# rashanarshad/deconv_api

Measured on AMD Instinct MI355X. Metric: images/sec, VGG16 deconv 224px (block5_conv3 deconvnet, top-4 mosaic), higher is better.
Workload: dtype bf16; 1 GPU; model=vgg16_deconvnet_block5_conv3, global_batch=256, seq_len=224, image_size=224, filters_per_image=4, parallelism=dp1

## Files before the change

deconv_api_amd/csrc/bindings.cpp:

```cpp
#include <torch/extension.h>
#include <ATen/hip/impl/HIPGuardImplMasqueradingAsCUDA.h>
#include <ATen/hip/impl/HIPStreamMasqueradingAsCUDA.h>

#include "jpeg_dec.h"
#include "jpeg_enc.h"
#include "kernels.h"

#include <cstdio>
#include <cstdlib>
#include <cstring>
#include <map>
#include <mutex>
#include <optional>

namespace {

using at::Tensor;

hipStream_t cur_stream() { return c10::hip::getCurrentHIPStreamMasqueradingAsCUDA().stream(); }

void check_cuda(const Tensor& t, const char* name) {
  TORCH_CHECK(t.is_cuda(), name, " must be a GPU tensor");
}

// ... 1329 lines not shown
  TORCH_CHECK(w.scalar_type() == at::kBFloat16 && w.is_contiguous() && w.dim() == 2 && w.size(0) == 64 &&
                  w.size(1) >= 576 && w.size(1) % 64 == 0,
              "conv_unpool_z: w bf16 [64, Kpad >= 576]");
  TORCH_CHECK(w2.scalar_type() == at::kBFloat16 && w2.is_contiguous() && w2.numel() == 32 * 64, "conv_unpool_z: w2 bf16 [32, 64]");
  check_cuda(code, "code");
  check_cuda(w, "w");
  check_cuda(w2, "w2");
  check_cuda(z, "z");
  dv::ConvArgs a{};
  a.N = (int)z.size(0); a.H = a.OH = (int)z.size(1); a.W = a.OW = (int)z.size(2); a.C = 64;
  a.OC = a.OCpad = 64; a.KH = a.KW = 3; a.stride = 1; a.pad_h = a.pad_w = 1;
  a.K = 576; a.Kpad = (int)w.size(1); a.M = a.N * a.H * a.W;
  a.relu = 1; a.relu_in = 1; a.code_div = (int)code_div; a.x_ld = 64; a.out_ld = 32;
  a.dtype = dv::DT_BF16;
  a.x = reinterpret_cast<const uint16_t*>(x.data_ptr());
  a.w = reinterpret_cast<const uint16_t*>(w.data_ptr());
  a.w2 = reinterpret_cast<const uint16_t*>(w2.data_ptr());
  a.code = code.data_ptr<uint8_t>();
  a.out = z.data_ptr();
  a.x_elems = avail_bytes(x) / 2;
  a.out_elems = avail_bytes(z) / 2;
  const int rc = dv::conv3x3_unpool_z_launch(a, cur_stream());
  if (rc == -4) return false;
  check_rc(rc, "conv_unpool_z");
  return true;
}

bool conv_stem_pool(Tensor x, Tensor w1, c10::optional<Tensor> b1, Tensor w2, c10::optional<Tensor> b2, Tensor out,
                    Tensor out_code) {
  check_cuda(x, "x");
  c10::hip::HIPGuardMasqueradingAsCUDA guard(x.device());
  TORCH_CHECK(x.dim() == 4 && x.scalar_type() == at::kBFloat16 && x.is_contiguous() && x.size(3) == 8,
              "conv_stem_pool: x bf16 [N, H, W, 8]");
  const int64_t N = x.size(0), H = x.size(1), W = x.size(2);
  TORCH_CHECK(H % 2 == 0 && W % 2 == 0, "conv_stem_pool: even H, W");
  TORCH_CHECK(out.dim() == 4 && out.scalar_type() == at::kBFloat16 && out.is_contiguous() && out.size(0) == N &&
                  out.size(1) == H / 2 && out.size(2) == W / 2 && out.size(3) == 64,
              "conv_stem_pool: out bf16 [N, H/2, W/2, 64]");
  TORCH_CHECK(out_code.scalar_type() == at::kByte && out_code.is_contiguous() && out_code.numel() == out.numel(),
              "conv_stem_pool: out_code u8 [N, H/2, W/2, 64]");
  TORCH_CHECK(w1.scalar_type() == at::kBFloat16 && w1.is_contiguous() && w1.dim() == 2 && w1.size(0) == 64 &&
                  w1.size(1) >= 96,
              "conv_stem_pool: w1 bf16 [64, Kpad >= 96]");
  TORCH_CHECK(w2.scalar_type() == at::kBFloat16 && w2.is_contiguous() && w2.dim() == 2 && w2.size(0) == 64 &&
                  w2.size(1) >= 576,
              "conv_stem_pool: w2 bf16 [64, Kpad >= 576]");
  for (const auto* b : {&b1, &b2})
    if (b->has_value())
      TORCH_CHECK((*b)->scalar_type() == at::kFloat && (*b)->is_contiguous() && (*b)->numel() >= 64 && (*b)->is_cuda(),
                  "conv_stem_pool: bias fp32 [>= 64] on the device");
  check_cuda(w1, "w1");
  check_cuda(w2, "w2");
  check_cuda(out, "out");
  check_cuda(out_code, "out_code");
  dv::ConvArgs a{};
  a.N = (int)N; a.H = a.OH = (int)H; a.W = a.OW = (int)W; a.C = 64;
  a.OC = a.OCpad = 64; a.KH = a.KW = 3; a.stride = 1; a.pad_h = a.pad_w = 1;
  a.K = 576; a.Kpad = (int)w2.size(1); a.M = (int)(N * H * W);
  a.relu = 1; a.code_div = 1; a.x_ld = 8; a.out_ld = 64;
  a.dtype = dv::DT_BF16;
  a.x = reinterpret_cast<const uint16_t*>(x.data_ptr());
  a.w = reinterpret_cast<const uint16_t*>(w2.data_ptr());
  a.bias = b2.has_value() ? b2->data_ptr<float>() : nullptr;
  a.w2 = reinterpret_cast<const uint16_t*>(w1.data_ptr());
  a.bias2 = b1.has_value() ? b1->data_ptr<float>() : nullptr;
  a.kpad2 = (int)w1.size(1);
  a.out = out.data_ptr();
  a.out_code = out_code.data_ptr<uint8_t>();
  a.x_elems = avail_bytes(x) / 2;
  a.out_elems = avail_bytes(out) / 2;
  dv::g_route = dv::ConvRoute{};
  const int rc = dv::conv3x3_stem_pool_launch(a, cur_stream());
  if (rc == -4) return false;
  check_rc(rc, "conv_stem_pool");
  return true;
}

void zsum3x3(Tensor z, Tensor out, c10::optional<Tensor> stats, int64_t stats_div) {
  check_cuda(z, "z");
  check_cuda(out, "out");
  c10::hip::HIPGuardMasqueradingAsCUDA guard(z.device());
  TORCH_CHECK(z.dim() == 4 && z.scalar_type() == at::kBFloat16 && z.is_contiguous() && z.size(3) == 32,
              "zsum3x3: z bf16 [N, H, W, 32]");
  TORCH_CHECK(out.scalar_type() == at::kFloat && out.is_contiguous() && out.numel() == z.numel() / 32 * 3,
              "zsum3x3: out fp32 [N, H, W, 3]");
  const int N = (int)z.size(0);
  double* st = nullptr;
  if (stats.has_value()) {
    check_cuda(*stats, "stats");
    TORCH_CHECK(stats->scalar_type() == at::kDouble && stats->is_contiguous() && stats_div >= 1 && N % stats_div == 0 &&
                    stats->numel() == 2 * (N / stats_div),
                "zsum3x3: stats fp64 [N/stats_div, 2]");
    check_rc((int)hipMemsetAsync(stats->data_ptr(), 0, stats->numel() * 8, cur_stream()), "stats memset");
    st = stats->data_ptr<double>();
  }
  check_rc(dv::zsum3x3_launch(reinterpret_cast<const uint16_t*>(z.data_ptr()), out.data_ptr<float>(), N,
                              (int)z.size(1), (int)z.size(2), st, (int)stats_div, cur_stream()),
           "zsum3x3");
}

void maxpool2x2(Tensor x, Tensor out, Tensor code) {
  check_cuda(x, "x");
  c10::hip::HIPGuardMasqueradingAsCUDA guard(x.device());
  TORCH_CHECK(x.dim() == 4 && is16(x) && x.is_contiguous(), "maxpool: x NHWC bf16 / fp16");
  const int64_t N = x.size(0), H = x.size(1), W = x.size(2), C = x.size(3);
  TORCH_CHECK(out.scalar_type() == x.scalar_type() && out.is_contiguous() && out.numel() == N * (H / 2) * (W / 2) * C,
              "maxpool: out");
  TORCH_CHECK(code.scalar_type() == at::kByte && code.is_contiguous() && code.numel() == out.numel(), "maxpool: code");
  check_rc(dv::maxpool2x2_launch(reinterpret_cast<const uint16_t*>(x.data_ptr()),
                                 reinterpret_cast<uint16_t*>(out.data_ptr()), code.data_ptr<uint8_t>(), (int)N, (int)H,
                                 (int)W, (int)C, f16(x), cur_stream()),
           "maxpool2x2");
}

void unpool2x2(Tensor p, Tensor code, Tensor out, int64_t code_div, bool relu) {
  check_cuda(p, "p");
  c10::hip::HIPGuardMasqueradingAsCUDA guard(p.device());
  TORCH_CHECK(out.dim() == 4 && is16(out) && out.is_contiguous(), "unpool: out NHWC bf16 / fp16");
  const int64_t N = out.size(0), H = out.size(1), W = out.size(2), C = out.size(3);
  TORCH_CHECK(p.scalar_type() == out.scalar_type() && p.is_contiguous() && p.numel() == N * (H / 2) * (W / 2) * C,
              "unpool: p");
  TORCH_CHECK(code_div >= 1 && N % code_div == 0, "unpool: code_div");
  TORCH_CHECK(code.scalar_type() == at::kByte && code.is_contiguous() && code.numel() == p.numel() / code_div,
              "unpool: code");
  check_rc(dv::unpool2x2_launch(reinterpret_cast<const uint16_t*>(p.data_ptr()), code.data_ptr<uint8_t>(),
                                reinterpret_cast<uint16_t*>(out.data_ptr()), (int)N, (int)H, (int)W, (int)C,
                                (int)code_div, relu ? 1 : 0, cur_stream()),
           "unpool2x2");
}


}

#ifndef DV_SOURCE_HASH
#define DV_SOURCE_HASH "unknown"
#endif
static const char kSourceHash[] = "DV_SOURCE_HASH:" DV_SOURCE_HASH;

PYBIND11_MODULE(TORCH_EXTENSION_NAME, m) {
  m.def("source_hash", [] { return std::string(kSourceHash + 15); }, "sha256 of the sources this binary was built from");
  m.def("subpixel_merge", &subpixel_merge, "strided-conv input gradient from its parity-class parts (+accumulate, emask)");
  m.def("sk_errors", &sk_errors, py::arg("reset") = false,
        "KW3P stream-K hand-offs that timed out since the last reset (their tiles are wrong)");
  m.doc() = "deconv_api_amd gfx950 (MI355X) HIP kernels";
  m.def("conv", &conv, "MFMA implicit-GEMM conv (fwd / unpool-gather / transposed; bf16/pool/f32 epilogues)",
        py::arg("x"), py::arg("w"), py::arg("bias"), py::arg("out"), py::arg("out_code"), py::arg("code"),
        py::arg("mask"), py::arg("geom"), py::arg("amode"), py::arg("epi"), py::arg("impl"),
        py::arg("res") = py::none(), py::arg("emask") = py::none(), py::arg("stats") = py::none(),
        py::arg("stats_div") = 1, py::arg("ucode") = py::none(), py::arg("ucode_div") = 1,
        py::arg("relu_cols") = 0, py::arg("out2") = py::none(), py::arg("split_col") = 0,
        py::arg("obits") = py::none(), py::arg("ebits") = py::none(), py::arg("w_kw3") = py::none());
  m.def("conv_route", &conv_route, "kernel the last conv call on this thread launched (route report)");
  m.def("misc_route", &misc_route, "kernel the last seed_deconv3x3 / maxpool2x2 / unpool2x2 / deprocess_mosaic call chose");
  m.def("conv_bpack", [] { return dv::g_route.bpack != 0; },
        "whether the last conv call on this thread staged its weights from the packed KW3 image (w_kw3)");
  m.def("conv_group_begin", &conv_group_begin, "start recording groupable small-problem convs (this thread)");
  m.def("conv_group_pause", [](bool p) { g_group_paused = p; }, "suspend / resume recording (dependent convs)");
  m.def("conv_group_end", &conv_group_end, "launch the recorded convs as grouped kernels; returns the launch count");
  m.def("dma_tune", [](int64_t cfg, int64_t ks) { dv::conv_dma_tune((int)cfg, (int)ks); },
        "force the LDS-DMA conv tile config / split-K factor (0 = automatic); tuning only");
  m.def("pool", &pool, "k x k max/avg pooling forward/backward", py::arg("in"), py::arg("out"), py::arg("idx"),
        py::arg("kind"), py::arg("dir"), py::arg("geom"), py::arg("bias") = py::none(), py::arg("relu") = false,
        py::arg("accumulate") = false);
  m.def("subpixel_scatter", &subpixel_scatter, "input gradient of a stride-s 1x1 conv from its GEMM result");
  m.def("sumsq_core", &sumsq_core, "DeepDream loss: per-image partial sums of squares over the core");
  m.def("stem_conv", &stem_conv, "strided few-channel stem conv (direct VALU kernels), fwd (dir 0) / dgrad (dir 1)");
  m.def("sumsq_core_bwd", &sumsq_core_bwd, "DeepDream loss gradient (+ optional addend)", py::arg("x"),
        py::arg("scale"), py::arg("gx"), py::arg("b"), py::arg("addend") = py::none(), py::arg("part") = py::none());
  m.def("tile_gather", &tile_gather, "tiled DeepDream: rolled tile gather into the 16-bit network input", py::arg("x"),
        py::arg("xin"), py::arg("plan"), py::arg("shift"), py::arg("rank"), py::arg("world"), py::arg("k0") = 0);
  m.def("tile_pack", &tile_pack, "tiled DeepDream: owned-pixel gradient pack + unit loss / sum|g| tail", py::arg("g"),
        py::arg("pack"), py::arg("plan"), py::arg("lpart"), py::arg("lcoef"), py::arg("ucap"), py::arg("rank"),
        py::arg("world"), py::arg("k0") = 0);
  m.def("tile_update", &tile_update, "tiled DeepDream: normalize + update the image from every rank's packs");
  m.def("tile_pack_elems", &tile_pack_elems);
  m.def("dream_update", &dream_update, "fused DeepDream normalize + update + next network input");
  m.def("octave_resize", &octave_resize, "DeepDream octave transition: corner-aligned bilinear resize of (a + b - c)",
        py::arg("a"), py::arg("b"), py::arg("c"), py::arg("y"), py::arg("yin") = py::none());
  m.def("stem7_fwd", &stem7_fwd, "ResNet-50 conv1 forward (7x7 / 2, RGB -> 64) on the tap-paired MFMA kernel");
  m.def("stem_dgrad_fused", &stem_dgrad_fused, "fused GEMM + col2im input gradient of a 7x7/2 RGB stem conv");
  m.def("col2im", &col2im, "col2im of a strided few-channel conv's input gradient");
  m.def("jpeg_data_urls", &jpeg_data_urls, "native JPEG + base64/quote data URLs (GIL released)");
  m.def("softmax_rows", &softmax_rows, "row softmax (classifier head)");
  m.def("paced_copy", &paced_copy, "bench: CU-occupying copy paced to a link bandwidth (all-gather interference model)");
  m.def("jpeg_gpu", &jpeg_gpu, "GPU baseline JPEG scans of uint8 [B,H,W,3] (restart per MCU row)");
  m.def("data_url_b64decode", &data_url_b64decode, "data URL payload -> bytes (lenient base64, GIL released)");
  m.def("url_unquote_plus", &url_unquote_plus, "unquote_plus of an ASCII str -> bytes (GIL released)");
  m.def("jpeg_gpu_header", &jpeg_gpu_header, "SOI..SOS of the GPU encoder's streams");
  m.def("jpeg_gpu_max_width", &dv::jpeg_gpu_max_width, "widest image the GPU encoder takes");
  m.def("jpeg_gpu_data_urls", &jpeg_gpu_data_urls, "GPU scans -> data URLs (host base64, GIL released)");
  m.def("jpeg_encode", &jpeg_encode, "native baseline JPEG encode (GIL released)");
  m.def("jpeg_parse_coeffs", &jpeg_parse_coeffs, "baseline JPEG bytes -> None | (header, int16 coefficients) (GIL released)");
  m.def("data_url_parse_coeffs", &data_url_parse_coeffs, "data URL -> (payload | None, None | parsed coefficients)");
  m.def("jpeg_dec_batch", &jpeg_dec_batch, "GPU JPEG decode of a batch: coefficients -> RGB, two launches");
  m.def("channel_sum", &channel_sum);
  m.def("topk_pos", &topk_pos);
  m.def("seed_deconv3x3", &seed_deconv3x3);
  m.def("seed_map", &seed_map, "deconvnet seed maps (all / max, optional max-unpool for pool targets)");
  m.def("deprocess_mosaic", &deprocess_mosaic, py::arg("recon"), py::arg("out"), py::arg("tiles"), py::arg("reverse"),
        py::arg("stats") = py::none());
  m.def("resize_preprocess", &resize_preprocess);
  m.def("resize_batch", &resize_batch, "variable-size batch resize (+preprocess) from one staged blob");
  m.def("preprocess_u8", &preprocess_u8, "resized RGB u8 -> caffe-preprocessed bf16 network input");
  m.def("maxpool2x2", &maxpool2x2);
  m.def("unpool2x2", &unpool2x2);
  m.def("conv_stem_pool", &conv_stem_pool, "fused VGG16 stem: conv 8->64 -> conv 64->64 -> 2x2 max-pool + switches");
  m.def("conv_unpool_z", &conv_unpool_z, "unpool -> conv3x3 64->64 -> ReLU -> per-tap products of the next 64->3 conv");
  m.def("zsum3x3", &zsum3x3, "9-tap shift-add of a per-tap product map (+ ReLU, per-image stats)");
  m.attr("ARCH") = "gfx950";
}
```

deconv_api_amd/csrc/conv_halo_stream.hip:

```cpp
#include "common.h"
#include "kernels.h"

#include <cstdlib>
#include <cstring>

namespace dv {

namespace {

constexpr int HS_TH = 16, HS_TW = 32;
constexpr int HS_HH = HS_TH + 2, HS_HW = HS_TW + 2;
constexpr int HS_PS = 80;
constexpr int HS_HSLOTS = HS_HH * HS_HW * 5;
constexpr int HS_HI = (HS_HSLOTS + 511) / 512;
constexpr int HS_HBUF = HS_HI * 8 * 1024;
constexpr uint32_t HS_OOB = 0x80000000u;

typedef int hs_i32x4 __attribute__((ext_vector_type(4)));

__device__ __forceinline__ void hs_dma16(const hs_i32x4& rsrc, const uint8_t* lds_dst, uint32_t voff) {
  asm volatile("s_mov_b32 m0, %0\n\ts_nop 0\n\tbuffer_load_dwordx4 %1, %2, 0 offen lds"
               :
               : "s"(__builtin_amdgcn_readfirstlane((uint32_t)(uintptr_t)lds_dst)), "v"(voff), "s"(rsrc)
               : "memory");
// ... 552 lines not shown
      issue_w(k + 2);
      const uint8_t* wb = ring + (k % RING) * BSLOT + wrd;
      const int kh = t / 3, kw = t % 3;
      v8 wf[FN], pf[4];
#pragma unroll
      for (int j = 0; j < FN; ++j) wf[j] = *reinterpret_cast<const v8*>(wb + j * 16 * 64);
#pragma unroll
      for (int i = 0; i < 4; ++i) {
        const int p = (4 * wave + i + kh) * H16_HW + px + kw;
        pf[i] = *reinterpret_cast<const v8*>(hb + p * 64 + ((q ^ h16_swz(p)) << 4));
      }
      __builtin_amdgcn_s_setprio(1);
#pragma unroll
      for (int i = 0; i < 4; ++i)
#pragma unroll
        for (int j = 0; j < FN; ++j) acc[i][j] = mfma16x16x32<DT>(wf[j], pf[i], acc[i][j]);
      __builtin_amdgcn_s_setprio(0);
      if constexpr (UNPOOL) {
        if (t == STEPS_PER_CHUNK - 1 && c + 1 < nch) {
          hs_wait<STEPS_PER_CHUNK * BI>();
          __builtin_amdgcn_s_barrier();
          expand((c + 1) & 1);
          asm volatile("s_waitcnt lgkmcnt(0)" ::: "memory");
        }
      }
    }
  }
  }
  hs_wait<0>();

  const int ox = tx0 + px;
  float4 bv[FN];
#pragma unroll
  for (int j = 0; j < FN; ++j)
    bv[j] = a.bias ? *reinterpret_cast<const float4*>(a.bias + 16 * j + 4 * q) : make_float4(0.f, 0.f, 0.f, 0.f);
  const float lo = a.relu ? 0.f : -INFINITY;
  uint16_t* out = reinterpret_cast<uint16_t*>(a.out);
  if constexpr (POOL) {
    const int PH = H >> 1, PW = W >> 1;
#pragma unroll
    for (int i = 0; i < 4; i += 2) {
      const long long prow = ((long long)n * PH + ((ty0 >> 1) + 2 * wave + (i >> 1))) * PW + (ox >> 1);
      const bool st = (px & 1) == 0;
#pragma unroll
      for (int j = 0; j < FN; ++j) {
        const int oc = 16 * j + 4 * q;
        const float b4[4] = {bv[j].x, bv[j].y, bv[j].z, bv[j].w};
        float best[4];
        uint32_t codes = 0;
#pragma unroll
        for (int r = 0; r < 4; ++r) {
          float w4[4];
#pragma unroll
          for (int d = 0; d < 2; ++d) {
            const float v = to_f<DT>(from_f<DT>(fmaxf(acc[i + d][j][r] + b4[r], lo)));
            w4[2 * d] = v;
            w4[2 * d + 1] = __int_as_float(__builtin_amdgcn_mov_dpp(__float_as_int(v), 0xB1, 0xF, 0xF, false));
          }
          float m = w4[0];
          uint32_t cc = 0;
#pragma unroll
          for (int e = 1; e < 4; ++e)
            if (w4[e] > m) {
              m = w4[e];
              cc = e;
            }
          best[r] = m;
          codes |= cc << (8 * r);
        }
        if (st && oc < a.OC && DV_BOUNDS(prow * a.out_ld + oc, 4, a.out_elems, "hs16 pool out")) {
          *reinterpret_cast<uint2*>(out + prow * a.out_ld + oc) =
              make_uint2(pack2<DT>(best[0], best[1]), pack2<DT>(best[2], best[3]));
          *reinterpret_cast<uint32_t*>(a.out_code + prow * a.OC + oc) = codes;
        }
      }
    }
    return;
  }
  if constexpr (LEPI) {
    __syncthreads();
    constexpr int ROWB = OCT * 2, CPR = OCT / 8;
    uint8_t* wreg = smem + wave * 64 * ROWB;
    static_assert(4 * 64 * ROWB <= (int)sizeof(smem), "LDS epilogue slices");
#pragma unroll
    for (int i = 0; i < 4; ++i)
#pragma unroll
      for (int j = 0; j < FN; ++j) {
        const float v0 = fmaxf(acc[i][j][0] + bv[j].x, lo), v1 = fmaxf(acc[i][j][1] + bv[j].y, lo);
        const float v2 = fmaxf(acc[i][j][2] + bv[j].z, lo), v3 = fmaxf(acc[i][j][3] + bv[j].w, lo);
        const int ch = 2 * j + (q >> 1);
        *reinterpret_cast<uint2*>(wreg + (i * 16 + px) * ROWB + ((ch ^ (px & (CPR - 1))) << 4) + (q & 1) * 8) =
            make_uint2(pack2<DT>(v0, v1), pack2<DT>(v2, v3));
      }
    asm volatile("s_waitcnt lgkmcnt(0)" ::: "memory");
    constexpr int PPI = 64 / CPR, NT = 64 / PPI;
    const int pc = lane % CPR;
    uint4 em[NT];
#pragma unroll
    for (int t = 0; t < NT; ++t) {
      const int lp = t * PPI + lane / CPR;
      const int lc = pc ^ (lp & (CPR - 1));
      const long long pix = ((long long)n * a.OH + ty0 + 4 * wave + (lp >> 4)) * a.OW + tx0 + (lp & 15);
      em[t] = make_uint4(0x3C003C00u, 0x3C003C00u, 0x3C003C00u, 0x3C003C00u);
      if (a.ebits && lc * 8 < a.OC)
        em[t].x = a.ebits[pix * a.ebits_ld + lc];
      else if (a.emask && lc * 8 < a.OC && DV_BOUNDS(pix * a.emask_ld + lc * 8, 8, a.emask_elems, "hs16 emask"))
        em[t] = *reinterpret_cast<const uint4*>(a.emask + pix * a.emask_ld + lc * 8);
    }
#pragma unroll
    for (int t = 0; t < NT; ++t) {
      const int lp = t * PPI + lane / CPR;
      const int lc = pc ^ (lp & (CPR - 1));
      const long long pix = ((long long)n * a.OH + ty0 + 4 * wave + (lp >> 4)) * a.OW + tx0 + (lp & 15);
      uint4 v = *reinterpret_cast<const uint4*>(wreg + lp * ROWB + pc * 16);
      if (a.ebits) {
        v = mask_bits8(v, em[t].x);
      } else if (a.emask) {
        v.x = mask_pos_pk(v.x, em[t].x);
        v.y = mask_pos_pk(v.y, em[t].y);
        v.z = mask_pos_pk(v.z, em[t].z);
        v.w = mask_pos_pk(v.w, em[t].w);
      }
      if (lc * 8 < a.OC && DV_BOUNDS(pix * a.out_ld + lc * 8, 8, a.out_elems, "hs16 out")) {
        *reinterpret_cast<uint4*>(out + pix * a.out_ld + lc * 8) = v;
        if (a.obits) a.obits[pix * a.obits_ld + lc] = (uint8_t)pos_bits8(v);
      }
    }
    return;
  }
#pragma unroll
  for (int i = 0; i < 4; ++i) {
    const int oy = ty0 + 4 * wave + i;
    const long long pix = ((long long)n * a.OH + oy) * a.OW + ox;
    uint16_t* orow = out + pix * a.out_ld;
    uint2 em[FN];
#pragma unroll
    for (int j = 0; j < FN; ++j) {
      const int oc = 16 * j + 4 * q;
      em[j] = make_uint2(0x3C003C00u, 0x3C003C00u);
      if (a.emask && oc < a.OC && DV_BOUNDS(pix * a.emask_ld + oc, 4, a.emask_elems, "hs16 emask"))
        em[j] = *reinterpret_cast<const uint2*>(a.emask + pix * a.emask_ld + oc);
    }
#pragma unroll
    for (int j = 0; j < FN; ++j) {
      const int oc = 16 * j + 4 * q;
      if (oc >= a.OC) continue;
      const float v0 = fmaxf(acc[i][j][0] + bv[j].x, lo), v1 = fmaxf(acc[i][j][1] + bv[j].y, lo);
      const float v2 = fmaxf(acc[i][j][2] + bv[j].z, lo), v3 = fmaxf(acc[i][j][3] + bv[j].w, lo);
      if (DV_BOUNDS(pix * a.out_ld + oc, 4, a.out_elems, "hs16 out"))
        *reinterpret_cast<uint2*>(orow + oc) =
            make_uint2(mask_pos_pk(pack2<DT>(v0, v1), em[j].x), mask_pos_pk(pack2<DT>(v2, v3), em[j].y));
    }
  }
}

static int hs_ring() {
  static int v = [] {
    const char* e = dv_ab_env("DV_HS_RING");
    const int r = e ? std::atoi(e) : 3;
    return r == 4 || r == 5 ? r : 3;
  }();
  return v;
}

#define HS_LAUNCH(DT_, OCT_, POOL_)                                                                    \
  do {                                                                                                 \
    if (ring == 5)                                                                                     \
      hipLaunchKernelGGL((conv3x3_hs_kernel<DT_, OCT_, POOL_, 5>), grid, block, 0, s, a, tx, ty);      \
    else if (ring == 4)                                                                                \
      hipLaunchKernelGGL((conv3x3_hs_kernel<DT_, OCT_, POOL_, 4>), grid, block, 0, s, a, tx, ty);      \
    else                                                                                               \
      hipLaunchKernelGGL((conv3x3_hs_kernel<DT_, OCT_, POOL_, 3>), grid, block, 0, s, a, tx, ty);      \
  } while (0)

int conv3x3_hs_launch(const ConvArgs& a, int epi, hipStream_t s, bool* lepi_used) {
  if (lepi_used) *lepi_used = false;
  if (dv_ab_env("DV_NO_HS") != nullptr) return -4;
  if ((a.OCpad == 192 || a.OCpad == 256) && a.OC > 128 && epi == CONV_E_BF16 && dv_ab_env("DV_NO_HS_SPLIT") == nullptr) {
    ConvArgs a1 = a, a2 = a;
    a1.OC = 128;
    a1.OCpad = 128;
    a2.OC = a.OC - 128;
    a2.OCpad = a.OCpad - 128;
    a2.w = a.w + (long long)128 * a.Kpad;
    a2.bias = a.bias ? a.bias + 128 : nullptr;
    a2.out = reinterpret_cast<uint16_t*>(a.out) + 128;
    a2.out_elems = a.out_elems - 128;
    if (a.emask) {
      a2.emask = a.emask + 128;
      a2.emask_elems = a.emask_elems - 128;
    }
    a1.obits = a2.obits = nullptr;
    a1.ebits = a2.ebits = nullptr;
    if (a2.OC % 4 != 0) return -4;
    const int r1 = conv3x3_hs_launch(a1, epi, s);
    if (r1 < 0) return r1;
    const int r2 = conv3x3_hs_launch(a2, epi, s);
    g_route.flags |= CR_F_OCSPLIT;
    return r2;
  }
  const bool geom = a.KH == 3 && a.KW == 3 && a.stride == 1 && a.pad_h == a.pad_w && a.pad_h >= 0 && a.pad_h <= 2 &&
                    a.OH == a.H + 2 * a.pad_h - 2 && a.OW == a.W + 2 * a.pad_w - 2 && a.OH > 0 && a.OW > 0;
  if (!geom || a.C % 32 != 0 || a.x_ld % 8 != 0 || (a.OCpad != 64 && a.OCpad != 128) || a.relu_in || a.accumulate ||
      a.mask || a.code || a.res || a.ws || a.stats || a.ucode || a.relu_cols > 0 || a.out_ld % 4 != 0 ||
      (reinterpret_cast<uintptr_t>(a.out) & 7) || (reinterpret_cast<uintptr_t>(a.x) & 15) ||
      (reinterpret_cast<uintptr_t>(a.bias) & 15) ||
      (a.emask && (a.emask_ld % 4 != 0 || (reinterpret_cast<uintptr_t>(a.emask) & 7))) ||
      (long long)a.Kpad < 9LL * a.C || (long long)a.H * a.W * a.x_ld * 2 > 0x7FFFFFF0LL)
    return -4;
  const bool pool = epi == CONV_E_POOL;
  if (!pool && epi != CONV_E_BF16) return -4;
  if (pool && (a.pad_h != 1 || a.emask || a.H % 2 || a.W % 2 || a.out_code == nullptr || a.OC % 4 ||
               a.dtype != DT_BF16 || (reinterpret_cast<uintptr_t>(a.out_code) & 3)))
    return -4;
  if (a.OH % 16 == 0 && a.OW % 16 == 0 && a.OC % 4 == 0 && dv_ab_env("DV_NO_HS16") == nullptr) {
    const int t16x = a.OW / 16, t16y = a.OH / 16;
    const long long n16 = (long long)a.N * t16x * t16y;
    if (n16 <= 0 || n16 > 0x7fffffffLL) return -2;
    const dim3 g16((unsigned)n16), b16(256);
#define HS16(DT_, OCT_, POOL_, LEPI_)                                                                            \
  hipLaunchKernelGGL((conv3x3_hs16_kernel<DT_, OCT_, POOL_, false, OCT_ == 64 ? 3 : 1, LEPI_>), g16, b16, 0, s, a, t16x, \
                     t16y)
    const char* he = dv_ab_env("DV_HS16_EPI");
    const bool lepi = !pool && !(he && std::strcmp(he, "reg") == 0) && a.OC % 8 == 0 && a.out_ld % 8 == 0 &&
                      !(reinterpret_cast<uintptr_t>(a.out) & 15) &&
                      (!a.emask || (a.emask_ld % 8 == 0 && !(reinterpret_cast<uintptr_t>(a.emask) & 15)));
    if (lepi_used) *lepi_used = lepi;
    route_set(CR_HS16, 0, a.OCpad, 0, 0, pool ? CR_E_POOL : (lepi ? CR_E_LDS : CR_E_REG));
    if (pool) {
      if (a.OCpad == 128) HS16(DT_BF16, 128, true, false);
      else HS16(DT_BF16, 64, true, false);
    } else if (a.dtype == DT_F16) {
      if (a.OCpad == 128) {
        if (lepi) HS16(DT_F16, 128, false, true);
        else HS16(DT_F16, 128, false, false);
      } else {
        if (lepi) HS16(DT_F16, 64, false, true);
        else HS16(DT_F16, 64, false, false);
      }
    } else {
      if (a.OCpad == 128) {
        if (lepi) HS16(DT_BF16, 128, false, true);
        else HS16(DT_BF16, 128, false, false);
      } else {
        if (lepi) HS16(DT_BF16, 64, false, true);
        else HS16(DT_BF16, 64, false, false);
      }
    }
#undef HS16
    return (int)hipGetLastError();
  }
  const int tx = (a.OW + HS_TW - 1) / HS_TW, ty = (a.OH + HS_TH - 1) / HS_TH;
  const long long nwg = (long long)a.N * tx * ty;
  if (nwg <= 0 || nwg > 0x7fffffffLL) return -2;
  const dim3 grid((unsigned)nwg), block(512);
  const int ring = hs_ring();
  const char* he = dv_ab_env("DV_HS16_EPI");
  const bool lepi = !pool && ring == 3 && !(he && std::strcmp(he, "reg") == 0) && a.OC % 8 == 0 && a.out_ld % 8 == 0 &&
                    !(reinterpret_cast<uintptr_t>(a.out) & 15) &&
                    (!a.emask || (a.emask_ld % 8 == 0 && !(reinterpret_cast<uintptr_t>(a.emask) & 15)));
  if (lepi_used) *lepi_used = lepi;
  route_set(CR_HS32, 0, a.OCpad, 0, 0, pool ? CR_E_POOL : (lepi ? CR_E_LDS : CR_E_REG));
#define HS_LEPI(DT_, OCT_, NB1_) \
  hipLaunchKernelGGL((conv3x3_hs_kernel<DT_, OCT_, false, 3, NB1_, true>), grid, block, 0, s, a, tx, ty)
  if (pool) {
    if (a.OCpad == 128) HS_LAUNCH(DT_BF16, 128, true);
    else HS_LAUNCH(DT_BF16, 64, true);
  } else if (a.C == 32 && a.OCpad == 64) {
    if (a.dtype == DT_F16) {
      if (lepi) HS_LEPI(DT_F16, 64, true);
      else hipLaunchKernelGGL((conv3x3_hs_kernel<DT_F16, 64, false, 3, true>), grid, block, 0, s, a, tx, ty);
    } else {
      if (lepi) HS_LEPI(DT_BF16, 64, true);
      else hipLaunchKernelGGL((conv3x3_hs_kernel<DT_BF16, 64, false, 3, true>), grid, block, 0, s, a, tx, ty);
    }
  } else if (lepi) {
    if (a.dtype == DT_F16) {
      if (a.OCpad == 128) HS_LEPI(DT_F16, 128, false);
      else HS_LEPI(DT_F16, 64, false);
    } else {
      if (a.OCpad == 128) HS_LEPI(DT_BF16, 128, false);
      else HS_LEPI(DT_BF16, 64, false);
    }
  } else if (a.dtype == DT_F16) {
    if (a.OCpad == 128) HS_LAUNCH(DT_F16, 128, false);
    else HS_LAUNCH(DT_F16, 64, false);
  } else {
    if (a.OCpad == 128) HS_LAUNCH(DT_BF16, 128, false);
    else HS_LAUNCH(DT_BF16, 64, false);
  }
#undef HS_LEPI
  return (int)hipGetLastError();
}

int conv3x3_stem_pool_launch(const ConvArgs& a, hipStream_t s) {
  if (a.KH != 3 || a.KW != 3 || a.stride != 1 || a.pad_h != 1 || a.pad_w != 1 || a.C != 64 || a.OC != 64 ||
      a.OCpad != 64 || a.x_ld != 8 || a.H != a.OH || a.W != a.OW || a.H % 16 || a.W % 16 || a.H <= 0 || a.W <= 0 ||
      a.N <= 0 || a.dtype != DT_BF16 || a.w2 == nullptr || a.kpad2 < 96 || a.Kpad < 9 * 64 || a.out_code == nullptr ||
      a.out_ld != 64 || a.relu != 1 || a.relu_in || a.accumulate || a.mask || a.code || a.res || a.emask || a.ws ||
      a.ucode || (reinterpret_cast<uintptr_t>(a.x) & 15) || (reinterpret_cast<uintptr_t>(a.out) & 7) ||
      (reinterpret_cast<uintptr_t>(a.out_code) & 3) || (reinterpret_cast<uintptr_t>(a.w2) & 15) ||
      (long long)a.H * a.W * 8 * 2 > 0x7FFFFFF0LL)
    return -4;
  const int tx = a.W / 16, ty = a.H / 16;
  const long long nwg = (long long)a.N * tx * ty;
  if (nwg > 0x7fffffffLL) return -2;
  route_set(CR_HS16, 0, 64, 0, 0, CR_E_POOL);
  g_route.cfg = 1;
  hipLaunchKernelGGL((conv3x3_hs16_kernel<DT_BF16, 64, true, false, 3, false, true>), dim3((unsigned)nwg), dim3(256), 0,
                     s, a, tx, ty);
  return (int)hipGetLastError();
}

}
```

deconv_api_amd/csrc/kernels.h:

```cpp
#pragma once
#include <hip/hip_runtime_api.h>
#include <stdint.h>

#include <cstdlib>

static inline bool dv_ablations_on() {
  const char* on = std::getenv("DV_ABLATIONS");
  return on != nullptr && on[0] == '1' && on[1] == 0;
}
static inline const char* dv_ab_env(const char* name) { return dv_ablations_on() ? std::getenv(name) : nullptr; }

namespace dv {

enum ConvAMode : int {
  CONV_A_FWD = 0,
  CONV_A_UNPOOL = 1,
  CONV_A_TRANSPOSE = 2,
};
enum ConvEpi : int {
  CONV_E_BF16 = 0,
  CONV_E_POOL = 1,
  CONV_E_F32 = 2,
};

enum { DT_BF16 = 0, DT_F16 = 1 };

struct ConvArgs {
  const uint16_t* x;
  long long x_ld;
  const uint16_t* mask;
  long long mask_ld;
  const uint8_t* code;
  int code_div;
  const uint16_t* w;
  const float* bias;
  void* out;
  long long out_ld;
  uint8_t* out_code;
  int N, H, W, C;
  int OH, OW, OC, OCpad;
  int KH, KW, stride, pad_h, pad_w;
  int K, Kpad;
  int M;
  int m_base;
  int relu, relu_in, accumulate;
  int dtype;
  const uint16_t* res;
  long long res_ld;
  const uint16_t* emask;
  long long emask_ld;
  int vec_epi;
  int epi_batch;
  float* ws;
  int ksplit;
  double* stats;
  int stats_div;
  const uint8_t* ucode;
  int ucode_div;
  long long x_elems, out_elems, res_elems, emask_elems;
  int relu_cols;
  void* out2;
  long long out2_ld;
  int split_col;
  long long out2_elems;
  const uint16_t* w2;
  int pool_t;
  float* skw;
  unsigned* skflag;
  int skslots;
  unsigned* skerr;
  uint8_t* obits;
  long long obits_ld;
  const uint8_t* ebits;
  long long ebits_ld;
  const float* bias2;
  int kpad2;
  const uint16_t* wp;
  long long wp_elems;
};
constexpr long long kSkSlotFloats = 256LL * 256LL;
constexpr int kSkMaxWg = 1024;

constexpr int kGroupMax = 4;
struct ConvGroup {
  ConvArgs p[kGroupMax];
  int start[kGroupMax + 1];
  int tiles_n[kGroupMax];
  int n;
};

enum ConvRouteKind : int {
  CR_NONE = 0, CR_IGEMM, CR_HALO_V1, CR_HALO_V2, CR_POOL_V3, CR_C8_STREAM, CR_HS16, CR_HS32, CR_PW, CR_DMA,
  CR_KW3, CR_KW3P, CR_GROUP,
};
enum ConvRouteEpi : int {
  CR_E_NONE = 0, CR_E_REG, CR_E_LDS, CR_E_UNPOOL, CR_E_POOL, CR_E_STRIPS, CR_E_PERSIST,
  CR_E_POOL_T, CR_E_POOL_LDS,
};
enum ConvRouteFlag : int {
  CR_F_SK = 1,
  CR_F_OCSPLIT = 2,
  CR_F_TAIL = 4,
  CR_F_UNPOOL = 8,
  CR_F_RELU_COPY = 16,
  CR_F_MASK = 32,
};
struct ConvRoute {
  int kind, bm, bn, stages, ksplit, epi, flags, m_base, cfg;
  int bpack;
};
extern __thread ConvRoute g_route;
static inline void route_set(int kind, int bm, int bn, int stages, int ksplit, int epi, int flags = 0) {
  g_route = ConvRoute{kind, bm, bn, stages, ksplit, epi, (g_route.flags & (CR_F_UNPOOL | CR_F_RELU_COPY)) | flags, 0, 0};
}

extern __thread const char* g_misc_route;

int conv_igemm_launch(const ConvArgs& a, int amode, int epi, hipStream_t stream);
int conv_dma_launch(const ConvArgs& a, int amode, int epi, hipStream_t stream);
int conv_dma_splitk(const ConvArgs& a);
void conv_dma_tune(int cfg, int ks);
int splitk_reduce_launch(const ConvArgs& a, int epi, hipStream_t stream);
int conv_dma_group_cfg(const ConvArgs& a, int amode, int epi);
int conv_dma_group_launch(const ConvArgs* ps, int n, int amode, int epi, hipStream_t stream);
int stem_conv_fwd_launch(const uint16_t* x, const float* w, const float* bias, uint16_t* y, int N, int H, int W,
                         int OH, int OW, int C, int cr, int cout, int k, int stride, int pad, int relu, long long x_ld,
                         long long y_ld, int dtype, hipStream_t s);
int stem_conv_dgrad_launch(const uint16_t* gy, const float* w, uint16_t* gx, int N, int H, int W, int OH, int OW,
                           int C, int cr, int cout, int k, int stride, int pad, long long gy_ld, long long gx_ld,
                           int dtype, hipStream_t s);
int conv_pw_launch(const ConvArgs& a, hipStream_t stream);

int channel_sum_launch(const uint16_t* x, float* sums, int N, int HW, int C, int f16, hipStream_t s);
int topk_pos_launch(const float* v, int* idx, float* val, int N, int C, int k, hipStream_t s);
int seed_deconv3x3_launch(const float* S, const int* f, const uint16_t* wt, uint16_t* out,
                          int B, int H, int W, int Cin, int F, int f16, hipStream_t s);
int deprocess_mosaic_launch(const float* recon, uint8_t* out, int B, int H, int W, int tiles,
                            int reverse_channels, hipStream_t s);
int recon_stats_launch(const float* x, double* stats, long long per_group, int groups, hipStream_t s);
int deprocess_apply_launch(const float* recon, const double* stats, uint8_t* out, int B, int H, int W, int tiles,
                           int reverse_channels, hipStream_t s);
int resize_preprocess_launch(const uint8_t* img, int B, int Hs, int Ws, uint16_t* out, int OH, int OW,
                             int Cpad, int mode, int f16, hipStream_t s);
int resize_batch_launch(const uint8_t* blob, const long long* table, int B, void* out, int OH, int OW, int Cpad,
                        int fmt, hipStream_t s);
int preprocess_u8_launch(const uint8_t* in, uint16_t* out, long long P, int Cpad, int f16, hipStream_t s);
int maxpool2x2_launch(const uint16_t* x, uint16_t* out, uint8_t* code, int N, int H, int W, int C,
                      int f16, hipStream_t s);
int seed_map_launch(const uint16_t* out4, const int* idx, const uint8_t* code, float* S, int BK, int K, int H, int W,
                    int C, int mode, int f16, hipStream_t s);
int unpool2x2_launch(const uint16_t* p, const uint8_t* code, uint16_t* out, int N, int H, int W,
                     int C, int code_div, int relu, hipStream_t s);

}

namespace dv {
int subpixel_merge_launch(const uint16_t* const* p, const int* hc, const int* wc, const int* ld, const uint16_t* emask,
                          uint16_t* gx, int N, int H, int W, int C, int s, int acc, int dtype, hipStream_t st);
int subpixel_scatter_launch(const uint16_t* E, const uint16_t* emask, uint16_t* gx, int N, int H, int W, int C, int OH,
                            int OW, int s, int dtype, hipStream_t st);
int pool_launch(int kind, int dir, const uint16_t* in, uint16_t* out, uint8_t* idx, int N, int H, int W, int C,
                int OH, int OW, int k, int s, int pad, int dtype, hipStream_t st, long long x_ld = 0,
                long long y_ld = 0, const float* bias = nullptr, int relu = 0, int acc = 0);
int dream_update_launch(const uint16_t* g, float* x, uint16_t* xin, float* gpart, int gparts, const float* lpart,
                        const float* lcoef, int L, int lparts, uint8_t* done, float* loss, float step, float max_loss,
                        int N, int H, int W, int dtype, hipStream_t s);
int octave_resize_launch(const float* a, const float* b, const float* c, float* y, uint16_t* yin, int N, int Hs, int Ws, int Hd, int Wd,
                         int dtype, hipStream_t s);
int tile_gather_launch(const float* x, uint16_t* xin, const int* plan, const int* shift, int units, int rank, int world,
                       int k0, int H, int W, int Th, int Tw, int dtype, hipStream_t s);
int tile_pack_launch(const uint16_t* g, uint16_t* pack, const int* plan, const float* lpart, const float* lcoef, int L,
                     int lparts, int units, int ucap, int rank, int world, int k0, int Th, int Tw, int dtype, hipStream_t s);
long long tile_pack_elems(int ucap, int Th, int Tw);
int tile_update_launch(const uint16_t* packs, long long pack_elems, int units_per_rank, const int* plan, int nunits,
                       const int* shift, float* x, uint8_t* done, float* loss, float step, float max_loss, int world,
                       int H, int W, int Th, int Tw, int dtype, hipStream_t s);
int sumsq_core_launch(const uint16_t* x, float* part, int parts, int N, int H, int W, int C, int b, int dtype,
                      hipStream_t s);
int sumsq_core_bwd_launch(const uint16_t* x, const float* scale, const uint16_t* addend, uint16_t* gx, int N, int H, int W, int C, int b,
                          int dtype, hipStream_t s);
int sumsq_core_fused_launch(const uint16_t* x, const float* scale, const uint16_t* addend, uint16_t* gx, float* part,
                            int parts, int N, int H, int W, int C, int b, int dtype, hipStream_t s);
struct Col2ImGeom {
  int N, H, W, OH, OW, KH, KW, stride, pad_h, pad_w, Cr, J_ld;
};
int col2im_launch(const uint16_t* cols, uint16_t* gx, const Col2ImGeom& g, int dtype, hipStream_t s);
struct StemDgradGeom {
  int N, H, W, OH, OW, C, KH, KW, stride, pad, Cr, w_rows, w_ld;
};
int stem7_fwd_launch(const uint16_t* x, const uint16_t* w, const float* bias, uint16_t* y, int N, int H, int W, int OH,
                     int OW, int relu, int dtype, hipStream_t s);
int stem_dgrad_fused_launch(const uint16_t* gy, const uint16_t* mask, const uint16_t* wb, uint16_t* gx,
                            const StemDgradGeom& g, int dtype, hipStream_t s);
long long jpeg_gpu_ws_bytes(int B, int H, int W);
long long jpeg_gpu_out_cap(int H, int W);
int jpeg_gpu_max_width();
int jpeg_gpu_launch(const uint8_t* rgb, int B, int H, int W, const void* tables, void* ws, uint8_t* packed,
                    long long* off, hipStream_t s);
int jpeg_dec_launch(uint8_t* blob, long long blob_bytes, const int* table, int B, int total_blocks, int total_items,
                    hipStream_t s);
int softmax_rows_launch(const float* x, float* y, int M, int N, hipStream_t s);
int paced_copy_launch(const void* src, long long src_bytes, void* dst, long long bytes, int channels, double gbs,
                      hipStream_t s);
int conv3x3_halo_launch(const ConvArgs& a, int unpool, int epi, hipStream_t s, bool* stats_done = nullptr);
int conv3x3_pool_v3_launch(const ConvArgs& a, hipStream_t s);
int conv3x3_unpool_z_launch(const ConvArgs& a, hipStream_t s);
int zsum3x3_launch(const uint16_t* z, float* out, int N, int H, int W, double* stats, int stats_div, hipStream_t s);
int conv3x3_c8_stream_launch(const ConvArgs& a, hipStream_t s);
int conv3x3_stem_pool_launch(const ConvArgs& a, hipStream_t s);
int conv3x3_hs_launch(const ConvArgs& a, int epi, hipStream_t s, bool* lepi_used = nullptr);
}
```

deconv_api_amd/knobs.py:

```python
from __future__ import annotations

import os
from typing import Optional

RUNTIME = {
    "DV_NO_KW3_SK": "stream-K off for KW3P convs (the recovery named by the hand-off timeout error, ops/conv.py)",
    "DV_POOL_SPLIT": "layers whose pool runs as a separate vectorized kernel (config 2 option, docs/KERNELS.md)",
    "DV_STEM_FUSE": "kill switch of the fused VGG16 stem (conv -> conv -> pool in one launch)",
    "DV_FUSED_TAIL": "kill switch of the fused deconvnet tail (unpool -> conv -> per-tap products)",
    "DV_CONV_IMPL": "conv kernel policy for tests / bring-up (auto | dma | igemm | halo)",
    "DV_CONV_GROUP": "grouped launch of independent small convs (DeepDream), 0 = per-conv launches",
    "DV_TILE_COLLECTIVE": "run the multi-rank tiled-DeepDream code path on a 1-rank RCCL group (rehearsal)",
    "DV_TILE_CHUNKS": "tile units per rank split into this many chunks whose all-gathers overlap compute",
    "DV_TILE_CHUNK_STREAMS": "streams the chunks of a tiled step fork onto",
    "DV_TILE_LOCAL_CHUNKS": "chunks per rank when the dream is not collective (one GPU)",
    "DV_TILE_CAPTURE_COLL": "capture the tiled octave's all-gathers inside its hipGraph (0: per-step graphs)",
    "DV_DREAM_GRAPHS": "hipGraph replay of DeepDream steps (0: eager, debugging)",
    "DV_DREAM_OCTAVE_GRAPH": "one hipGraph per octave incl. all steps (0: one graph per step)",
    "DV_FAULT": "fault injection for the failover tests (utils/faults.py)",
    "DV_ROCTX": "roctx ranges around engine stages (utils/tracing.py)",
    "DV_MAX_PIXELS": "decoded-pixel cap of a request image (codec/image.py)",
    "DV_FORCE_PG": "create a real process group at world 1 (exercises RCCL collectives on one GPU)",
    "DV_INGEST_DIR": "directory of the front-end <-> GPU-owner Unix sockets (serve/ingest.py)",
    "DV_ABLATIONS": "honour the ABLATION switches below (tools / variant tests only)",
}

ABLATION = {
    "DV_KW3": "KW3 kernel off / forced, ahead of the small-problem tiles too (tests: small shapes with many borders)",
    "DV_KW3_VAR": "KW3 main-loop variant (profiles/kw3_variants_r3.txt, kw3_staging_ablation_r5.txt)",
    "DV_KW3_TILE": "KW3P tile shape (profiles/kw3_ab_r4.txt)",
    "DV_KW3_SK": "stream-K on every eligible grid, not only short ones (profiles/kw3_skall_ab_r5.txt)",
    "DV_KW3P_EPI": "register-layout 8-B epilogue instead of the LDS-staged 16-B one (profiles/kw3_epi_ab_r5.txt)",
    "DV_KW3_BPACK": "0: KW3 weights from the strided w_gemm, not the packed image (profiles/kw3_bpack_ab_r7.txt)",
    "DV_KW3P_NO_PRE": "no step-1 DMA ahead of the epilogue (profiles/kw3_pre_ab_r5.txt)",
    "DV_KW3P_UNP_NT": "plain instead of non-temporal unpool stores (profiles/bench_c2_r5_unp_nt_ab.txt)",
    "DV_NO_KW3P_UNPOOL": "unpool-out conv-downs off KW3P (profiles/kw3_store_ablation_r5.txt)",
    "DV_ALLOW_WRONG_ABLATION": "timing-only variants whose outputs are wrong (tools/kw3_ab.py, tools/tail_ab.py)",
    "DV_NO_AUTO_CFG": "size-based DMA tile choice only (docs/KERNELS.md)",
    "DV_SMALL_TILE_KMIN": "K threshold of the 64x64 small-problem tile",
    "DV_NO_SPLITK": "split-K off, latched at the first DMA conv (tools/small_conv_latency.py; tests: dma_tune(0, 1))",
    "DV_NO_SMALL_SPLITK": "small-problem split-K off",
    "DV_SMALL_SPLITK_MN": "M x N ceiling of the small-problem split-K",
    "DV_NO_POOL_T": "per-element pool-epilogue stores (profiles/bench_c2_r4_pool_t_ab.txt)",
    "DV_POOL_EPI": "pool epilogue variant (profiles/bench_c2_r5_pool_epi_ab.txt)",
    "DV_NO_VEC_EPI": "scalar conv epilogue",
    "DV_NO_EPI_BATCH": "per-row epilogue batching off (profiles/dream_c3_r2_epi_batch*.log)",
    "DV_NO_C8_STREAM": "first-layer row-streaming kernel off",
    "DV_HS_MIN_W": "smallest map side routed to the halo-stream kernels",
    "DV_HS_EMASK_OFF": "masked dgrads back on the DMA kernel",
    "DV_HS_PAD_OFF": "pad != 1 convs off the halo-stream kernels",
    "DV_NO_HS": "halo-stream kernels off",
    "DV_NO_HS16": "16x16-tile halo-stream kernel off",
    "DV_NO_HS_SPLIT": "192/256-channel convs not split into halo-stream halves",
    "DV_HS_RING": "halo-stream ring depth",
    "DV_HS16_EPI": "register-layout epilogue of hs16 (profiles/bench_c2_r5_hs16_epi_ab.txt)",
    "DV_TAIL_V": "fused-tail schedule bits (profiles/bench_c2_r5_tail_v_ab.txt)",
    "DV_STREAM_P": "row-streaming kernel prefetch depth",
    "DV_NO_POOL_UNROLL": "generic k x k pooling loop (profiles/dream_r4_maxpool_bwd_s2_ab.txt)",
    "DV_NO_PW": "persistent 1x1 kernel off (tools/pw_bench.py)",
    "DV_PW_MIN_TILES": "tiles below which 1x1 convs stay on the DMA kernel (profiles/dream_r4_pw_min_tiles.txt)",
    "DV_PW_WG_PER_CU": "persistent 1x1 workgroups per CU",
    "DV_NO_STREAM_PROBE": "plain pool streams instead of probed / high-priority ones (runtime/streams.py)",
    "DV_DREAM_OCTAVE_RESIZE": "torch octave resize instead of the HIP kernel (profiles/dream_c3_r4_octave_resize_ab.txt)",
    "DV_DREAM_FUSED": "fused step tail off",
    "DV_DREAM_FUSED_LOSS": "fused loss off",
    "DV_DREAM_TAPS": "tap-split stride-2 dgrads (profiles/dream_c5_r2_taps.log)",
    "DV_DREAM_SPLIT": "concurrent sub-batches per DeepDream batch (profiles/dream_c3_split_sweep_r2.txt)",
    "DV_RELU_BITS": "1-bit ReLU masks off (profiles/dream_c5_r5_relu_bits_ab.txt)",
    "DV_SUBPIXEL": "sub-pixel scatter for stride-2 1x1 dgrads (profiles/kstats_c5_r2_subpixel.txt)",
    "DV_STEM_FUSED": "InceptionV3 stem fusion (profiles/dream_c3_r2_stem*.log)",
    "DV_STEM_DIRECT": "direct stride-2 stem gradient (profiles/dream_c5_r3_stem_ab.txt)",
    "DV_STEM7": "ResNet conv1 tap-paired kernel (profiles/dream_c5_r5_stem7_ab.txt)",
    "DV_COL2IM": "LDS-tiled col2im of the RGB stem gradient",
    "DV_STRIDED_DIRECT_GFLOP": "size threshold of the direct strided dgrad",
    "DV_MERGE_B1": "merged Inception branch-head GEMMs (profiles/dream_c3_r2_merge_b1.txt)",
    "DV_INCEPTION_FUSED": "one-node Inception blocks (profiles/dream_c3_merged.log)",
}

BUILD = {
    "DV_HIP_CHECK": "launch-status check macro (csrc/common.h), not an environment variable",
    "DV_DEBUG": "-DDV_DEBUG=1 build: device bounds checks (python -m deconv_api_amd._build --debug)",
    "DV_BOUNDS": "the bounds-check macro of DV_DEBUG builds (csrc/common.h)",
    "DV_SOURCE_HASH": "sha256 of csrc + flags embedded in _C (_build.py provenance)",
    "DV_OFFLOAD_ARCH": "offload arch of the in-tree build (gfx950)",
    "DV_AUTOBUILD": "ops/native.py: build (or rebuild a stale) _C in-tree on first use",
    "DV_SKIP_PROVENANCE": "ops/native.py: load a _C built from other sources (scratch builds in tools)",
    "DV_S": "kernel-local macro (conv_smalln.hip), not an environment variable",
    "DV_S2": "kernel-local macro (conv_smalln.hip), not an environment variable",
    "DV_P": "kernel-local macro (conv_smalln.hip), not an environment variable",
}


def config_names():
    import dataclasses

    from .config import Config

    return {"DV_" + f.name.upper() for f in dataclasses.fields(Config)}


def ablations_on() -> bool:
    return os.environ.get("DV_ABLATIONS", "") == "1"


def ablation(name: str, default: Optional[str] = None) -> Optional[str]:
    assert name in ABLATION, f"{name} is not a registered ablation switch (knobs.py)"
    return os.environ.get(name, default) if ablations_on() else default
```

Measured before the change: 7905 images/s.

## Add persistent fused stem conv kernel that prefetches next tile's RGB and weights

Adds a persistent version of the fused VGG stem (conv1_1 + conv1_2 + 2x2 maxpool with codes). The grid is capped at two workgroups per CU, and each workgroup walks many tiles. The first-layer weights and biases stay in registers across tiles. The next tile's RGB halo and the weight ring are DMA-prefetched while the current tile computes. This is meant to cut per-workgroup setup and the launch tail, at the cost of a fixed grid and larger LDS use. It is on by default unless bias2 is misaligned or the DV_HS16_PERSIST env var is 0.

```diff
diff --git a/deconv_api_amd/csrc/bindings.cpp b/deconv_api_amd/csrc/bindings.cpp
--- a/deconv_api_amd/csrc/bindings.cpp
+++ b/deconv_api_amd/csrc/bindings.cpp
@@ -1505,6 +1505,8 @@
         py::arg("obits") = py::none(), py::arg("ebits") = py::none(), py::arg("w_kw3") = py::none());
   m.def("conv_route", &conv_route, "kernel the last conv call on this thread launched (route report)");
   m.def("misc_route", &misc_route, "kernel the last seed_deconv3x3 / maxpool2x2 / unpool2x2 / deprocess_mosaic call chose");
+  m.def("conv_route_flags", [] { return dv::g_route.flags; },
+        "ConvRouteFlag bits of the last conv / conv_stem_pool call on this thread (64: the persistent fused stem)");
   m.def("conv_bpack", [] { return dv::g_route.bpack != 0; },
         "whether the last conv call on this thread staged its weights from the packed KW3 image (w_kw3)");
   m.def("conv_group_begin", &conv_group_begin, "start recording groupable small-problem convs (this thread)");
diff --git a/deconv_api_amd/csrc/conv_halo_stream.hip b/deconv_api_amd/csrc/conv_halo_stream.hip
--- a/deconv_api_amd/csrc/conv_halo_stream.hip
+++ b/deconv_api_amd/csrc/conv_halo_stream.hip
@@ -728,6 +728,212 @@
             make_uint2(mask_pos_pk(pack2<DT>(v0, v1), em[j].x), mask_pos_pk(pack2<DT>(v2, v3), em[j].y));
     }
   }
+}
+
+namespace {
+constexpr int SP_BSLOT = 64 * 64 * 3;
+constexpr int SP_RGB = 2 * 4 * 1024;
+constexpr int SP_SMEM = 2 * H16_HBUF + 2 * SP_BSLOT + SP_RGB;
+static_assert(SP_SMEM <= 80 * 1024, "persistent stem: 2 workgroups per CU");
+}
+
+__global__ void __launch_bounds__(256, 2) conv3x3_stem_persist_kernel(const ConvArgs a, int tiles_x, int tiles_y, int ntiles) {
+  constexpr int DT = DT_BF16;
+  constexpr int C = 64, FN = 4;
+  typedef typename Vec8<DT>::type v8;
+  __shared__ __attribute__((aligned(16))) uint8_t smem[SP_SMEM];
+  uint8_t* halo = smem;
+  uint8_t* ring = smem + 2 * H16_HBUF;
+  uint8_t* rgb = ring + 2 * SP_BSLOT;
+
+  const int tid = threadIdx.x, lane = tid & 63;
+  const int wave = __builtin_amdgcn_readfirstlane(tid >> 6);
+  const int q = lane >> 4, px = lane & 15;
+  const int H = a.H, W = a.W;
+  const int per_img = tiles_x * tiles_y;
+  const int G = (int)gridDim.x;
+  int tile = xcd_remap(blockIdx.x, G);
+  if (tile >= ntiles) return;
+
+  const long long img = (long long)H * W * 8;
+  const hs_i32x4 wr = hs_rsrc(a.w, (long long)a.OCpad * a.Kpad * 2);
+  uint32_t woff[3];
+#pragma unroll
+  for (int u = 0; u < 3; ++u) {
+    const int s = wave * 64 + lane;
+    const int r = s >> 2, ch = (s & 3) ^ h16_swz(s >> 2);
+    woff[u] = (uint32_t)(((long long)r * a.Kpad + u * C + ch * 8) * 2);
+  }
+  auto issue_w = [&](int k, bool real) {
+    const int c = k / 3, t = k - 3 * (k / 3);
+    const uint32_t add = (uint32_t)((t * 3 * C + c * 32) * 2);
+    uint8_t* dst = ring + (k & 1) * SP_BSLOT;
+#pragma unroll
+    for (int u = 0; u < 3; ++u) hs_dma16(wr, dst + (u * 4 + wave) * 1024, real ? woff[u] + add : HS_OOB);
+  };
+  auto issue_rgb = [&](int T) {
+    const bool real = T < ntiles;
+    const int n = real ? T / per_img : 0;
+    const int tr = real ? T - n * per_img : 0;
+    const int ty0 = (tr / tiles_x) * H16_T, tx0 = (tr % tiles_x) * H16_T;
+    const hs_i32x4 xr = hs_rsrc(a.x + (long long)n * img, img * 2);
+#pragma unroll
+    for (int u = 0; u < 2; ++u) {
+      const int e = (u * 4 + wave) * 64 + lane;
+      const int ry = e / 20, rx = e - 20 * (e / 20);
+      const int y = ty0 - 2 + ry, x = tx0 - 2 + rx;
+      const bool ok = real && e < 400 && (unsigned)y < (unsigned)H && (unsigned)x < (unsigned)W;
+      hs_dma16(xr, rgb + (u * 4 + wave) * 1024, ok ? (uint32_t)((y * W + x) * 16) : HS_OOB);
+    }
+  };
+
+  issue_rgb(tile);
+  issue_w(0, true);
+  v8 wa[3][4];
+#pragma unroll
+  for (int s = 0; s < 3; ++s)
+#pragma unroll
+    for (int j = 0; j < 4; ++j)
+      wa[s][j] = *reinterpret_cast<const v8*>(a.w2 + (long long)(j * 16 + px) * a.kpad2 + s * 32 + q * 8);
+  f32x4 b1[4];
+#pragma unroll
+  for (int j = 0; j < 4; ++j)
+    b1[j] = a.bias2 ? *reinterpret_cast<const f32x4*>(a.bias2 + j * 16 + q * 4) : f32x4{0.f, 0.f, 0.f, 0.f};
+  f32x4 bv[FN];
+#pragma unroll
+  for (int j = 0; j < FN; ++j)
+    bv[j] = a.bias ? *reinterpret_cast<const f32x4*>(a.bias + 16 * j + 4 * q) : f32x4{0.f, 0.f, 0.f, 0.f};
+#pragma unroll
+  for (int s = 0; s < 3; ++s)
+#pragma unroll
+    for (int j = 0; j < 4; ++j) asm volatile("" : "+v"(wa[s][j]));
+#pragma unroll
+  for (int j = 0; j < 4; ++j) asm volatile("" : "+v"(b1[j]), "+v"(bv[j]));
+  hs_wait<0>();
+  __builtin_amdgcn_s_barrier();
+
+  const float lo = a.relu ? 0.f : -INFINITY;
+  uint16_t* out = reinterpret_cast<uint16_t*>(a.out);
+  const int PH = H >> 1, PW = W >> 1;
+  const int wrd = px * 64 + ((q ^ h16_swz(px)) << 4);
+  for (;;) {
+    const int n = tile / per_img;
+    const int tr = tile - n * per_img;
+    const int ty0 = (tr / tiles_x) * H16_T, tx0 = (tr % tiles_x) * H16_T;
+    const int next = tile + G;
+    const bool more = next < ntiles;
+
+    for (int f = wave; f < 21; f += 4) {
+      const int p = f * 16 + px;
+      const int hy = p / H16_HW, hx = p - H16_HW * (p / H16_HW);
+      f32x4 c1[4];
+#pragma unroll
+      for (int j = 0; j < 4; ++j) c1[j] = f32x4{0.f, 0.f, 0.f, 0.f};
+#pragma unroll
+      for (int s = 0; s < 3; ++s) {
+        const int t = 4 * s + q;
+        const int kh = t / 3, kw = t - 3 * (t / 3);
+        uint4 xv = make_uint4(0u, 0u, 0u, 0u);
+        if (t < 9 && p < H16_HW * H16_HW) xv = *reinterpret_cast<const uint4*>(rgb + ((hy + kh) * 20 + hx + kw) * 16);
+#pragma unroll
+        for (int j = 0; j < 4; ++j) c1[j] = mfma16x16x32<DT>(wa[s][j], __builtin_bit_cast(v8, xv), c1[j]);
+      }
+      if (p < H16_HW * H16_HW) {
+        const int y = ty0 - 1 + hy, x = tx0 - 1 + hx;
+        const bool in = (unsigned)y < (unsigned)H && (unsigned)x < (unsigned)W;
+#pragma unroll
+        for (int j = 0; j < 4; ++j) {
+          float v[4];
+#pragma unroll
+          for (int r = 0; r < 4; ++r) v[r] = in ? fmaxf(c1[j][r] + b1[j][r], 0.f) : 0.f;
+          const int ch = (j & 1) * 2 + (q >> 1);
+          *reinterpret_cast<uint2*>(halo + (j >> 1) * H16_HBUF + p * 64 + ((ch ^ h16_swz(p)) << 4) + (q & 1) * 8) =
+              make_uint2(pack_bf2(v[0], v[1]), pack_bf2(v[2], v[3]));
+        }
+      }
+    }
+    asm volatile("s_waitcnt lgkmcnt(0)" ::: "memory");
+
+    f32x4 acc[4][FN];
+#pragma unroll
+    for (int i = 0; i < 4; ++i)
+#pragma unroll
+      for (int j = 0; j < FN; ++j) acc[i][j] = f32x4{0.f, 0.f, 0.f, 0.f};
+#pragma unroll
+    for (int c = 0; c < 2; ++c) {
+      const uint8_t* hb = halo + c * H16_HBUF;
+#pragma unroll
+      for (int kh = 0; kh < 3; ++kh) {
+        const int k = c * 3 + kh;
+        if (k == 1) hs_wait<2>();
+        else hs_wait<0>();
+        __builtin_amdgcn_s_barrier();
+        if (k < 5) issue_w(k + 1, true);
+        else issue_w(0, more);
+        if (k == 0) issue_rgb(next);
+        const uint8_t* wb = ring + (k & 1) * SP_BSLOT + wrd;
+#pragma unroll
+        for (int kw = 0; kw < 3; ++kw) {
+          v8 wf[FN], pf[4];
+#pragma unroll
+          for (int j = 0; j < FN; ++j) wf[j] = *reinterpret_cast<const v8*>(wb + kw * 64 * 64 + j * 16 * 64);
+#pragma unroll
+          for (int i = 0; i < 4; ++i) {
+            const int p = (4 * wave + i + kh) * H16_HW + px + kw;
+            pf[i] = *reinterpret_cast<const v8*>(hb + p * 64 + ((q ^ h16_swz(p)) << 4));
+          }
+          __builtin_amdgcn_s_setprio(1);
+#pragma unroll
+          for (int i = 0; i < 4; ++i)
+#pragma unroll
+            for (int j = 0; j < FN; ++j) acc[i][j] = mfma16x16x32<DT>(wf[j], pf[i], acc[i][j]);
+          __builtin_amdgcn_s_setprio(0);
+        }
+      }
+    }
+    __builtin_amdgcn_s_barrier();
+
+    const int ox = tx0 + px;
+#pragma unroll
+    for (int i = 0; i < 4; i += 2) {
+      const long long prow = ((long long)n * PH + ((ty0 >> 1) + 2 * wave + (i >> 1))) * PW + (ox >> 1);
+      const bool st = (px & 1) == 0;
+#pragma unroll
+      for (int j = 0; j < FN; ++j) {
+        const int oc = 16 * j + 4 * q;
+        float best[4];
+        uint32_t codes = 0;
+#pragma unroll
+        for (int r = 0; r < 4; ++r) {
+          float w4[4];
+#pragma unroll
+          for (int d = 0; d < 2; ++d) {
+            const float v = to_f<DT>(from_f<DT>(fmaxf(acc[i + d][j][r] + bv[j][r], lo)));
+            w4[2 * d] = v;
+            w4[2 * d + 1] = __int_as_float(__builtin_amdgcn_mov_dpp(__float_as_int(v), 0xB1, 0xF, 0xF, false));
+          }
+          float m = w4[0];
+          uint32_t cc = 0;
+#pragma unroll
+          for (int e = 1; e < 4; ++e)
+            if (w4[e] > m) {
+              m = w4[e];
+              cc = e;
+            }
+          best[r] = m;
+          codes |= cc << (8 * r);
+        }
+        if (st && oc < a.OC && DV_BOUNDS(prow * a.out_ld + oc, 4, a.out_elems, "stem persist pool out")) {
+          *reinterpret_cast<uint2*>(out + prow * a.out_ld + oc) =
+              make_uint2(pack2<DT>(best[0], best[1]), pack2<DT>(best[2], best[3]));
+          *reinterpret_cast<uint32_t*>(a.out_code + prow * a.OC + oc) = codes;
+        }
+      }
+    }
+    if (!more) break;
+    tile = next;
+  }
+  hs_wait<0>();
 }
 
 static int hs_ring() {
@@ -869,6 +1075,15 @@
   return (int)hipGetLastError();
 }
 
+static int hs_num_cus() {
+  static int n = [] {
+    int dev = 0, cu = 256;
+    if (hipGetDevice(&dev) != hipSuccess || hipDeviceGetAttribute(&cu, hipDeviceAttributeMultiprocessorCount, dev) != hipSuccess) cu = 256;
+    return cu > 0 ? cu : 256;
+  }();
+  return n;
+}
+
 int conv3x3_stem_pool_launch(const ConvArgs& a, hipStream_t s) {
   if (a.KH != 3 || a.KW != 3 || a.stride != 1 || a.pad_h != 1 || a.pad_w != 1 || a.C != 64 || a.OC != 64 ||
       a.OCpad != 64 || a.x_ld != 8 || a.H != a.OH || a.W != a.OW || a.H % 16 || a.W % 16 || a.H <= 0 || a.W <= 0 ||
@@ -883,6 +1098,15 @@
   if (nwg > 0x7fffffffLL) return -2;
   route_set(CR_HS16, 0, 64, 0, 0, CR_E_POOL);
   g_route.cfg = 1;
+  const char* pe = dv_ab_env("DV_HS16_PERSIST");
+  if (!(pe && std::atoi(pe) == 0) && !(reinterpret_cast<uintptr_t>(a.bias2) & 15)) {
+    const char* ge = dv_ab_env("DV_HS16_GRID");
+    long long grid = ge ? std::atoll(ge) : 0;
+    if (grid <= 0 || grid > 0x7fffffffLL) grid = 2LL * hs_num_cus() < nwg ? 2LL * hs_num_cus() : nwg;
+    g_route.flags |= CR_F_PERSIST;
+    hipLaunchKernelGGL(conv3x3_stem_persist_kernel, dim3((unsigned)grid), dim3(256), 0, s, a, tx, ty, (int)nwg);
+    return (int)hipGetLastError();
+  }
   hipLaunchKernelGGL((conv3x3_hs16_kernel<DT_BF16, 64, true, false, 3, false, true>), dim3((unsigned)nwg), dim3(256), 0,
                      s, a, tx, ty);
   return (int)hipGetLastError();
diff --git a/deconv_api_amd/csrc/kernels.h b/deconv_api_amd/csrc/kernels.h
--- a/deconv_api_amd/csrc/kernels.h
+++ b/deconv_api_amd/csrc/kernels.h
@@ -104,6 +104,7 @@
   CR_F_UNPOOL = 8,
   CR_F_RELU_COPY = 16,
   CR_F_MASK = 32,
+  CR_F_PERSIST = 64,
 };
 struct ConvRoute {
   int kind, bm, bn, stages, ksplit, epi, flags, m_base, cfg;
diff --git a/deconv_api_amd/knobs.py b/deconv_api_amd/knobs.py
--- a/deconv_api_amd/knobs.py
+++ b/deconv_api_amd/knobs.py
@@ -54,6 +54,8 @@
     "DV_NO_HS_SPLIT": "192/256-channel convs not split into halo-stream halves",
     "DV_HS_RING": "halo-stream ring depth",
     "DV_HS16_EPI": "register-layout epilogue of hs16 (profiles/bench_c2_r5_hs16_epi_ab.txt)",
+    "DV_HS16_PERSIST": "0: fused stem as one workgroup per tile, not the persistent kernel (profiles/stem_persist_ab_r8.txt)",
+    "DV_HS16_GRID": "workgroups of the persistent fused stem (tests: small shapes walk many tiles per workgroup)",
     "DV_TAIL_V": "fused-tail schedule bits (profiles/bench_c2_r5_tail_v_ab.txt)",
     "DV_STREAM_P": "row-streaming kernel prefetch depth",
     "DV_NO_POOL_UNROLL": "generic k x k pooling loop (profiles/dream_r4_maxpool_bwd_s2_ab.txt)",
```

Result: no change. 7984 images/s, median of 6 (+1.0%).
